# Qw11111111111/SequenceAligning

Hardware: AMD Instinct MI355X
Metric: GCUPS (affine-gap NW) at 1/2/4/8 MI355X; % of HBM roofline (higher is better)
Workload: dtype i32-exact (i16x2 packed arithmetic)

## Files before the change

### sequencealigning_amd/csrc/nw_host.cpp

```cpp
#include <hip/hip_runtime.h>

#include <algorithm>
#include <cstdlib>
#include <array>
#include <cstring>
#include <map>
#include <numeric>
#include <string>
#include <thread>
#include <unordered_set>
#include <vector>

#include "nw_host.hpp"

namespace saln {

Scoring scoring_or_default(const saln_nw_scoring *s) {
    if (!s) return Scoring{5, -4, -8, -6};
    return Scoring{s->match, s->mismatch, s->gap_open, s->gap_extend};
}

bool scores_fit_i32(const Scoring &s, uint64_t lq, uint64_t ld) {
    auto a = [](int64_t v) { return v < 0 ? -v : v; };
    const int64_t step = std::max({a(s.match), a(s.mismatch), a(s.gap_open) + a(s.gap_extend)});
// ... 225 lines not shown
        }
    return SALN_OK;
}

}

int saln::plan_create(saln_context *ctx, const uint64_t *q_off, uint64_t n_q,
                      const uint64_t *db_off, uint64_t n_db, const uint32_t *pair_q,
                      const uint32_t *pair_db, uint64_t n_pairs, int32_t mode,
                      const saln_nw_scoring *scoring, bool full_codes, saln_nw_plan **out) {
    if (!ctx || !q_off || !db_off || !out) return SALN_E_INVALID;
    *out = nullptr;
    if (mode != SALN_MODE_GLOBAL) {
        set_error("not implemented");
        return SALN_NOT_IMPLEMENTED;
    }
    const PairIndex pairs{pair_q, pair_db, n_q, n_db};
    if (!pairs.complete(n_pairs) || n_pairs > 0xFFFFFFFFull) return SALN_E_INVALID;
    HIP_TRY(hipSetDevice(ctx->device));
    const Options opts = ctx->opts.effective();
    StageClock clk(opts);
    auto *p = new saln_nw_plan;
    p->ctx = ctx;
    p->opts = opts;
    p->sc = scoring_or_default(scoring);
    p->full_codes = full_codes;
    const bool nib_on = !full_codes;
    const bool narrow = nib_on;
    for (int v = 0; v < kNumVariants; ++v) p->nib[v] = nib_on && variant_nib(v);
    p->n_pairs = n_pairs;
    p->cigar_off.resize(n_pairs + 1);
    std::vector<NwPairDesc> descs(n_pairs);
    uint64_t cig = 0;
    uint64_t memo_lq = ~0ull, memo_ld = ~0ull;
    bool memo_fit = false;
    int memo_var = 0;
    for (uint64_t k = 0; k < n_pairs; ++k) {
        uint64_t qi, di, lq, ld;
        if (!pairs.at(k, &qi, &di) ||
            !pair_lengths(q_off, db_off, qi, di, 0x7FFFFFFFull, &lq, &ld)) {
            delete p;
            return SALN_E_INVALID;
        }
        NwPairDesc &d = descs[k];
        std::memset(&d, 0, sizeof(d));
        d.q_off = q_off[qi];
        d.db_off = db_off[di];
        if (lq != memo_lq || ld != memo_ld) {
            memo_lq = lq;
            memo_ld = ld;
            memo_fit = scores_fit_i32(p->sc, lq, ld);
            memo_var = memo_fit ? choose_variant((uint32_t)lq, (uint32_t)ld, p->sc, narrow) : 0;
        }
        if (!memo_fit) {
            delete p;
            set_error("pair too long for these penalties: its scores could leave the engine's "
                      "int32 range");
            return SALN_E_INVALID;
        }
        d.len_q = (uint32_t)lq;
        d.len_db = (uint32_t)ld;
        d.pair_id = (uint32_t)k;
        d.variant = (uint32_t)memo_var;
        d.cigar_off = cig;
        p->cigar_off[k] = cig;
        cig += lq + ld;
        p->cells += lq * ld;
    }
    p->cigar_off[n_pairs] = cig;
    clk.mark("plan: descs");
    {
        const uint64_t v8_min = (uint64_t)opts[Opt::WideMinPairs];
        uint64_t wide = 0;
        for (const NwPairDesc &d : descs)
            wide += d.variant == (uint32_t)kWidePackedVariant && d.len_q > 512;
        if (wide && wide < v8_min)
            for (NwPairDesc &d : descs)
                if (d.variant == (uint32_t)kWidePackedVariant && d.len_q > 512)
                    d.variant = (uint32_t)kStripeVariant;
    }
    std::vector<uint64_t> skey(n_pairs);
    for (uint64_t k = 0; k < n_pairs; ++k) {
        const NwPairDesc &d = descs[k];
        const bool empty = d.len_q == 0 || d.len_db == 0;
        const uint64_t nch = empty ? 0 : variant_geom((int)d.variant).n_chunks(d.len_q);
        skey[k] = (uint64_t)(empty ? (uint32_t)kNumVariants : d.variant) << 56 |
                  ((~nch) & 0xFFFFFFull) << 32 | (uint32_t)~d.len_db;
    }
    std::vector<uint32_t> order;
    const bool in_order = std::is_sorted(skey.begin(), skey.end());
    if (in_order) {
        p->h_pairs = std::move(descs);
    } else {
        order.resize(n_pairs);
        std::iota(order.begin(), order.end(), 0u);
        std::sort(order.begin(), order.end(), [&](uint32_t a, uint32_t b) {
            return skey[a] != skey[b] ? skey[a] < skey[b] : a < b;
        });
        p->h_pairs.resize(n_pairs);
    }
    clk.mark("plan: sort");
    uint64_t soff = 0, ooff = 0;
    for (uint64_t r = 0; r < n_pairs; ++r) {
        NwPairDesc d = in_order ? p->h_pairs[r] : descs[order[r]];
        const bool empty = d.len_q == 0 || d.len_db == 0;
        if (!empty) {
            const Geom g = variant_geom((int)d.variant);
            d.ops_off = ooff;
            ooff += (d.len_q + d.len_db + 9) / 10 + 1;
            if (g.n_chunks(d.len_q) > 1 || d.variant == kStripeVariant) {
                soff = (soff + 3) & ~3ull;
                d.scratch_off = soff;
                soff += (uint64_t)(d.variant == kStripeVariant ? kStripeSubMax * g.n_chunks(d.len_q)
                                                                : 1) *
                        scratch_col(d.len_db);
            }
            if (p->var_count[d.variant] == 0) p->var_first[d.variant] = (uint32_t)r;
            p->var_count[d.variant]++;
            p->var_maxld[d.variant] = std::max(p->var_maxld[d.variant], d.len_db);
            p->n_fill++;
        }
        p->h_pairs[r] = d;
    }
    {
        uint64_t waves = 0, cols = 0, waves_k1 = 0;
        bool free_all = true;
        for (uint32_t r = 0; r < p->var_count[kStripeVariant]; ++r) {
            const NwPairDesc &d = p->h_pairs[p->var_first[kStripeVariant] + r];
            waves += variant_geom(kStripeVariant).n_chunks(d.len_q);
            waves_k1 += (d.len_q + 63) / 64;
            cols += d.len_q;
            free_all = free_all && sentinel_free(p->sc, d.len_q, d.len_db);
        }
        const bool wide = p->var_count[kStripeVariant] &&
                          cols / p->var_count[kStripeVariant] >= 3000;
        p->stripe_pk = waves > 0 && free_all && stripe_packed(p->sc, waves, wide, opts);
        p->stripe_rows = p->stripe_pk ? 0 : stripe_rows_k(waves_k1, opts);
        p->stripe_sub = p->stripe_rows ? 4u / (uint32_t)p->stripe_rows : 1u;
        if (p->stripe_sub != kStripeSubMax) {
            uint64_t so = 0;
            for (uint64_t r = 0; r < p->n_fill; ++r) {
                NwPairDesc &d = p->h_pairs[r];
                const Geom g = variant_geom((int)d.variant);
                if (g.n_chunks(d.len_q) > 1 || d.variant == kStripeVariant) {
                    so = (so + 3) & ~3ull;
                    d.scratch_off = so;
                    so += (uint64_t)(d.variant == kStripeVariant ? p->stripe_sub * g.n_chunks(d.len_q) : 1) *
                          scratch_col(d.len_db);
                }
            }
            soff = so;
        }
    }
    uint64_t moff = 0;
    for (int v = 0; v < kNumVariants; ++v) {
        const Geom g = variant_geom(v);
        const uint64_t lb = p->nib[v] ? g.LBn() : g.LB();
        for (uint32_t a = p->var_first[v], e = a + p->var_count[v]; a < e; a += 64) {
            const uint32_t np = std::min<uint32_t>(64, e - a);
            uint64_t rows = 0, nbm = 0, own = 0;
            for (uint32_t s = 0; s < np; ++s) {
                const NwPairDesc &d = p->h_pairs[a + s];
                rows = std::max<uint64_t>(rows, d.len_db);
                nbm = std::max<uint64_t>(nbm, g.n_blocks(d.len_q));
                own += (uint64_t)d.len_db * g.n_blocks(d.len_q) * lb;
            }
            const uint64_t packed = rows * nbm * np * lb;
            if (v == kStripeVariant) {
                const bool pk = p->stripe_pk;
                for (uint32_t s = 0; s < np; ++s) {
                    NwPairDesc &d = p->h_pairs[a + s];
                    d.mask_off = moff;
                    d.mask_rs = g.W();
                    d.mask_bs = pk ? 0u : (uint32_t)lb;
                    d.mask_cs = ((uint64_t)d.len_db + (pk ? 2 * g.G : g.G) - 1) * g.W();
                    moff += g.n_chunks(d.len_q) * d.mask_cs;
                }
            } else if (4 * packed <= 5 * own + 4096) {
                for (uint32_t s = 0; s < np; ++s) {
                    NwPairDesc &d = p->h_pairs[a + s];
                    d.mask_off = moff + s * lb;
                    d.mask_bs = (uint32_t)(np * lb);
                    d.mask_rs = nbm * np * lb;
                    d.mask_cs = (uint64_t)g.G * d.mask_bs;
                }
                moff += (packed + 255) & ~255ull;
            } else {
                for (uint32_t s = 0; s < np; ++s) {
                    NwPairDesc &d = p->h_pairs[a + s];
                    d.mask_off = moff;
                    d.mask_bs = (uint32_t)lb;
                    d.mask_rs = g.n_blocks(d.len_q) * lb;
                    d.mask_cs = (uint64_t)g.G * lb;
                    moff += ((uint64_t)d.len_db * d.mask_rs + 255) & ~255ull;
                }
            }
        }
    }
    {
        p->sync_ev.resize(3);
        for (auto &e : p->sync_ev) {
            if (hipEventCreateWithFlags(&e, hipEventDisableTiming) != hipSuccess) {
                e = nullptr;
                set_error("hipEventCreate");
                saln_nw_plan_destroy(p);
                return SALN_E_HIP;
            }
        }
    }
    clk.mark("plan: layout");
    p->plan_index.resize(n_pairs);
    for (uint64_t r = 0; r < n_pairs; ++r) p->plan_index[p->h_pairs[r].pair_id] = (uint32_t)r;
    p->mask_bytes = moff;
    p->scratch_elems = soff;
    auto fail = [&](hipError_t e, const char *what) {
        set_error(std::string(what) + ": " + hipGetErrorString(e));
        saln_nw_plan_destroy(p);
        return SALN_E_HIP;
    };
    hipError_t e;
    if (n_pairs) {
        if ((e = dev_alloc(p->ctx, (void **)&p->d_pairs, n_pairs * sizeof(NwPairDesc))) != hipSuccess)
            return fail(e, "hipMalloc(pairs)");
        clk.mark("plan: pairs alloc");
        {
            std::lock_guard<std::mutex> lk(p->ctx->staging_mu);
            void *st = nullptr;
            const size_t nb = n_pairs * sizeof(NwPairDesc);
            if ((e = pinned_staging(p->ctx, nb, &st)) != hipSuccess) return fail(e, "pinned staging");
            std::memcpy(st, p->h_pairs.data(), nb);
            if ((e = hipMemcpy(p->d_pairs, st, nb, hipMemcpyHostToDevice)) != hipSuccess)
                return fail(e, "hipMemcpy(pairs)");
        }
        if ((e = dev_alloc(p->ctx, (void **)&p->d_endh, n_pairs * sizeof(int32_t))) != hipSuccess)
            return fail(e, "hipMalloc(end)");
    }
    clk.mark("plan: pairs h2d");
    if (moff && (e = dev_alloc(p->ctx, (void **)&p->d_mask, moff + 64)) != hipSuccess)
        return fail(e, "hipMalloc(mask workspace)");
    {
        std::vector<uint2> work;
        p->work_first.assign(n_pairs + 1, 0);
        for (uint64_t r = 0; r < n_pairs; ++r) {
            NwPairDesc &d = p->h_pairs[r];
            p->work_first[r] = (uint32_t)work.size();
            if (d.variant != (uint32_t)kStripeVariant || !d.len_q || !d.len_db) continue;
            const uint32_t nch = variant_geom(kStripeVariant).n_chunks(d.len_q);
            d.reserved = (uint32_t)p->n_prog;
            p->n_prog += nch;
            for (uint32_t ch = 0; ch < nch; ++ch) work.push_back(make_uint2((uint32_t)r, ch));
        }
        p->work_first[n_pairs] = (uint32_t)work.size();
        if (!work.empty()) {
            if ((e = dev_alloc(p->ctx, (void **)&p->d_work, work.size() * sizeof(uint2))) != hipSuccess ||
                (e = hipMemcpy(p->d_work, work.data(), work.size() * sizeof(uint2),
                               hipMemcpyHostToDevice)) != hipSuccess ||
                (e = dev_alloc(p->ctx, (void **)&p->d_prog, p->n_prog * sizeof(uint32_t))) != hipSuccess ||
                (e = dev_alloc(p->ctx, (void **)&p->d_err, kErrWords * sizeof(uint32_t))) != hipSuccess ||
                (e = hipMemset(p->d_err, 0, kErrWords * sizeof(uint32_t))) != hipSuccess ||
                (e = hipMemcpy(p->d_err, std::array<uint32_t, 2>{0u, kWaitLimitDefault}.data(),
                               2 * sizeof(uint32_t), hipMemcpyHostToDevice)) != hipSuccess)
                return fail(e, "stripe work list");
            if ((e = hipMemcpy(p->d_pairs, p->h_pairs.data(), n_pairs * sizeof(NwPairDesc),
                               hipMemcpyHostToDevice)) != hipSuccess)
                return fail(e, "hipMemcpy(pairs)");
        }
    }
    clk.mark("plan: mask+work");
    if (soff && (e = dev_alloc(p->ctx, (void **)&p->d_scratch, soff * sizeof(int2))) != hipSuccess)
        return fail(e, "hipMalloc(scratch)");
    p->ops_words = ooff;
    if (ooff && (e = dev_alloc(p->ctx, (void **)&p->d_ops, ooff * sizeof(uint32_t))) != hipSuccess)
        return fail(e, "hipMalloc(op stream)");
    if ((p->var_count[kNarrowVariant] && p->nib[kNarrowVariant]) || (p->var_count[7] && p->nib[7]) ||
        (p->full_codes && (p->var_count[5] || p->var_count[7]))) {
        if ((e = dev_alloc(p->ctx, (void **)&p->d_bail[0], kBailBytes)) != hipSuccess ||
            (e = hipMemset(p->d_bail[0], 0, kBailBytes)) != hipSuccess)
            return fail(e, "table fill bail words");
    }
    {
        const int passes = (int)opts[Opt::SpecPasses];
        const uint32_t nv = p->var_count[kStripeVariant];
        std::vector<SpecPair> sp;
        std::vector<uint2> blocks;
        if (opts[Opt::Spec] != 0 && passes > 0 && nv && nv <= kSpecMaxPairs) {
            for (uint32_t r = p->var_first[kStripeVariant]; r < p->var_first[kStripeVariant] + nv; ++r) {
                const NwPairDesc &d = p->h_pairs[r];
                const uint32_t S = (d.len_q + 255) / 256;
                if (S < kSpecMinStripes || S > kSpecMaxStripes) continue;
                sp.push_back(SpecPair{r, S, (uint32_t)blocks.size(), 0});
                for (uint32_t s = 0; s < S; ++s) blocks.push_back(make_uint2((uint32_t)sp.size() - 1, s));
            }
        }
        if (!sp.empty()) {
            p->spec_pairs = (uint32_t)sp.size();
            p->spec_blocks = (uint32_t)blocks.size();
            p->spec_passes = passes;
            p->spec_strict = opts[Opt::SpecStrict] != 0;
            if ((e = dev_alloc(p->ctx, (void **)&p->d_spec_blocks, blocks.size() * sizeof(uint2))) != hipSuccess ||
                (e = hipMemcpy(p->d_spec_blocks, blocks.data(), blocks.size() * sizeof(uint2),
                               hipMemcpyHostToDevice)) != hipSuccess ||
                (e = dev_alloc(p->ctx, (void **)&p->d_spec_pairs, sp.size() * sizeof(SpecPair))) != hipSuccess ||
                (e = hipMemcpy(p->d_spec_pairs, sp.data(), sp.size() * sizeof(SpecPair),
                               hipMemcpyHostToDevice)) != hipSuccess ||
                (e = dev_alloc(p->ctx, (void **)&p->d_spec_stripes, blocks.size() * sizeof(SpecStripe))) != hipSuccess ||
                (e = dev_alloc(p->ctx, (void **)&p->d_spec_ops,
                               blocks.size() * kSpecOpsCap * sizeof(uint32_t))) != hipSuccess ||
                (e = dev_alloc(p->ctx, (void **)&p->d_spec_done, n_pairs * sizeof(uint32_t))) != hipSuccess ||
                (e = hipMemset(p->d_spec_done, 0, n_pairs * sizeof(uint32_t))) != hipSuccess)
                return fail(e, "speculative walk tables");
        }
    }
    *out = p;
    return SALN_OK;
}

extern "C" {

int saln_nw_plan_info(const saln_nw_plan *p, uint64_t *mask_bytes, uint64_t *cigar_words,
                      uint64_t *cells) {
    if (!p) return SALN_E_INVALID;
    if (mask_bytes) *mask_bytes = p->mask_bytes;
    if (cigar_words) *cigar_words = p->cigar_off.back();
    if (cells) *cells = p->cells;
    return SALN_OK;
}

int saln_nw_cigar_offsets(const saln_nw_plan *p, uint64_t *off) {
    if (!p || !off) return SALN_E_INVALID;
    std::memcpy(off, p->cigar_off.data(), p->cigar_off.size() * sizeof(uint64_t));
    return SALN_OK;
}

int saln_nw_plan_set_timing(saln_nw_plan *p, int enable) {
    if (!p) return SALN_E_INVALID;
    HIP_TRY(hipSetDevice(p->ctx->device));
    if (p->ev_used) {
        const int rc = p->resolve_events();
        if (rc != SALN_OK) return rc;
    }
    p->timing = enable != 0;
    p->ktime.clear();
    constexpr size_t kEventSets = 64;
    while (p->timing && p->ev_pool.size() < kEventSets) {
        std::array<hipEvent_t, 4> e4{};
        for (auto &e : e4) HIP_TRY(hipEventCreate(&e));
// ... 544 lines not shown
```

### sequencealigning_amd/csrc/nw_kernels.hip

```cpp
#include <hip/hip_runtime.h>

#include <algorithm>
#include <atomic>
#include <cstdlib>
#include <type_traits>
#include <utility>

#include "nw_common.hpp"
#include "nw_host.hpp"
#include "saln_options.hpp"
#include "saln.h"

namespace saln {
bool stripe_packed(const Scoring &sc, uint64_t n_waves, bool wide, const Options &o);
}

namespace saln {

template <int G>
__device__ __forceinline__ int32_t shr1(int32_t old, int32_t v) {
    static_assert(G == 16 || G == 64, "group must be a DPP row or the wave");
    if constexpr (G == 16)
        return __builtin_amdgcn_update_dpp(old, v, 0x111 , 0xf, 0xf, false);
    else
// ... 58 lines not shown
        if (st == kStM) {
            if (i == 0 && j == 0) { ev = kEvOrigin; break; }
            if (i == 0 || j == 0) { ev = kEvDead; break; }
            const bool eq = q ? q[j - 1] == d[i - 1] : (mc.byte(i, j) >> 7) != 0;
            op = eq ? SALN_CIGAR_EQ : SALN_CIGAR_X;
            const uint8_t a = mc.argmax(i - 1, j - 1);
            --i;
            --j;
            st = (a & kArgD) ? kStD : ((a & kArgI) ? kStI : kStM);
        } else if (st == kStI) {
            if (j == 0) { ev = i >= 1 ? kEvPanic : kEvDead; break; }
            if (i == 0) { ev = kEvDead; break; }
            op = SALN_CIGAR_I;
            const uint8_t b = mc.ibits(i, j);
            --j;
            st = (b & 2) ? kStM : kStI;
        } else {
            if (i == 0) { ev = j >= 1 ? kEvPanic : kEvDead; break; }
            if (j == 0) { ev = kEvDead; break; }
            op = SALN_CIGAR_D;
            const uint8_t b = mc.dbits(i, j);
            --i;
            st = (b & 2) ? kStM : kStD;
        }
        if (op == run_op && run_len) {
            ++run_len;
        } else {
            if (run_len && out) out[nops] = (run_len << 4) | run_op;
            nops += run_len ? 1 : 0;
            run_op = op;
            run_len = 1;
        }
    }
    if (run_len) {
        if (out) out[nops] = (run_len << 4) | run_op;
        ++nops;
    }
    if (ev != kEvOrigin) nops = 0;
    if (out) {
        for (uint32_t a = 0, b = nops ? nops - 1 : 0; a < b; ++a, --b) {
            const uint32_t tmp = out[a];
            out[a] = out[b];
            out[b] = tmp;
        }
    }
    return WalkOut{ev, nops};
}

__device__ WalkOut walk_first(const MaskCell &mc, uint32_t es, uint32_t ld, uint32_t lq,
                              const uint8_t *q, const uint8_t *d, uint32_t *out) {
    WalkOut w{kEvDead, 0};
    while (es) {
        const int st = first_end_state(es);
        w = walk_greedy(mc, st, ld, lq, q, d, out);
        if (w.ev != kEvDead) break;
        es = end_states_after(es, st);
    }
    return w;
}

__device__ __forceinline__ saln_nw_result make_result(int32_t hend, WalkOut w, uint32_t es) {
    saln_nw_result r;
    r.score = hend >> 1;
    r.status = (hend & 1) ? SALN_REF_PANIC_BOUNDARY : SALN_OK;
    r.cigar_len = w.nops;
    r.end_states = (uint8_t)es;
    r.printed = w.ev == kEvOrigin ? 1 : 0;
    r.flags = (w.ev == kEvPanic && !(hend & 1)) ? 2 : 0;
    r.reserved = 0;
    return r;
}

__device__ __forceinline__ void walk_pair(const NwPairDesc &p, int32_t hend,
                                       const uint8_t *__restrict__ qs,
                                       const uint8_t *__restrict__ ds,
                                       const uint8_t *__restrict__ mask, Geom geo,
                                       saln_nw_result *__restrict__ results,
                                       uint32_t *__restrict__ cigar, Scoring sc) {
    const uint32_t lq = p.len_q, ld = p.len_db;
    const MaskCell mc{mask + p.mask_off, geo, p.mask_rs, p.mask_bs, p.mask_cs, sc};
    const uint8_t es = ld == 0 ? argmax_row0(sc, lq)
                     : lq == 0 ? argmax_col0(sc, ld) : (mc.byte(ld, lq) & 7);
    const WalkOut w = walk_first(mc, es, ld, lq, qs + p.q_off, ds + p.db_off,
                                 cigar ? cigar + p.cigar_off : nullptr);
    results[p.pair_id] = make_result(hend, w, es);
}

constexpr uint32_t kOpsPerWord = 10;

template <int K, bool kNib = false, uint32_t kCols = 0>
struct WalkGeo {
    static constexpr uint32_t LB = kNib ? 4 * ((K + 3) / 4 / 2 + 1) : (K + 3) / 4 * 4;
    static constexpr uint32_t NW = 2;
    static constexpr uint32_t W = K < 16 || kNib ? 4 : 8;
    static constexpr uint32_t SB = LB == 12 ? 12 : 16;
    static constexpr uint32_t kSlotBytes = 64 * 16;
    static constexpr uint32_t kWinBytes = W * kSlotBytes;
    static constexpr uint32_t QC = kNib ? (15 + kCols + 15) / 16 : 0;
    static constexpr uint32_t kWaveLds = NW * kWinBytes + QC * kSlotBytes;
    static constexpr uint32_t kVmcnt = NW * (W - 1);
    static_assert(LB <= 16, "LDS window slots hold 16 bytes per lane");
    static_assert((NW == 2 || NW == 3) && W >= 2 && W <= 8, "8 valid bits per window");
    static_assert(!kNib || kCols > 0, "4-bit walk: the variant's query width");
};

typedef __attribute__((address_space(3))) uint8_t lds_u8;

__device__ __forceinline__ uint32_t lds_off(const lds_u8 *p) { return (uint32_t)(uintptr_t)p; }

__device__ __forceinline__ void counted_store(uint32_t *ptr, uint32_t v) {
    asm volatile("global_store_dword %0, %1, off" : : "v"(ptr), "v"(v) : "memory");
}

__host__ __device__ constexpr uint32_t next_state_raw(uint32_t st, uint32_t f) {
    const uint32_t pr = f ^ 7u;
    return st == 0 ? ((pr & 2) ? kStD : (pr & 1) ? kStI : kStM)
         : st == 1 ? ((pr & 2) ? kStM : kStI)
         : st == 2 ? ((pr & 2) ? kStM : kStD)
                   : ((pr & 4) ? kStD : (pr & 1) ? kStM : kStI);
}
__host__ __device__ constexpr uint64_t make_next_lut() {
    uint64_t l = 0;
    for (uint32_t st = 0; st < 4; ++st)
        for (uint32_t f = 0; f < 8; ++f) l |= (uint64_t)next_state_raw(st, f) << (16 * st + 2 * f);
    return l;
}
constexpr uint64_t kNextLut = make_next_lut();

typedef uint32_t u32x4 __attribute__((ext_vector_type(4)));
template <uint32_t N>
__device__ __forceinline__ u32x4 window_seg(uint32_t addr) {
    static_assert(N < 64, "vmcnt immediate");
    u32x4 v;
    asm volatile("s_waitcnt vmcnt(%2)\n\tds_read_b128 %0, %1\n\ts_waitcnt lgkmcnt(0)"
                 : "=v"(v) : "v"(addr), "n"(N) : "memory");
    return v;
}

template <typename F, uint32_t... I>
__device__ __forceinline__ void unroll_each(F &&f, std::integer_sequence<uint32_t, I...>) {
    (f(std::integral_constant<uint32_t, I>{}), ...);
}

template <int G, int K, bool kNib = false>
__device__ void walk_pack_lds(const NwPairDesc &p, int32_t hend, const uint8_t *__restrict__ mask,
                              uint32_t *__restrict__ ops_all, saln_nw_result *__restrict__ results,
                              uint32_t *__restrict__ cigar, Scoring sc, lds_u8 *win,
                              const uint8_t *__restrict__ qs) {
    using WG = WalkGeo<K, kNib, G * K>;
    constexpr Geom geo{G, K};
    constexpr uint32_t kW = WG::W, NW = WG::NW;
    constexpr uint32_t kWin = WG::kWinBytes, kSlot = WG::kSlotBytes;
    constexpr uint64_t kMask30 = (1u << 30) - 1u;
    const uint64_t rs = p.mask_rs, cs = p.mask_cs;
    const uint32_t bs = p.mask_bs;
    const uint8_t *__restrict__ m = mask + p.mask_off;
    uint32_t *out = cigar ? cigar + p.cigar_off : nullptr;
    uint32_t *const ops = ops_all + p.ops_off;
    auto boff = [&](uint32_t b) __attribute__((always_inline)) {
        if constexpr (kNib) return (uint64_t)(b * bs);
        else return (uint64_t)(b / G) * cs + (uint64_t)((b % G) * bs);
    };
    uint64_t acc = 0;
    uint32_t sh = 0, wi = 0;
    uint32_t ti = p.len_db, tj = p.len_q;
    uint32_t sidx = 3u * 16u, lsh = 0;
    uint32_t walking = 1;
    uint32_t B = (tj - 1) / K, col = (tj - 1) % K;
    uint32_t wc = B % NW;
    uint32_t valid = NW == 3 ? 0xFFFFFFu : 0xFFFFu;
    uint64_t ow0 = 0, ow1 = 0, ow2 = 0;
    auto set_ow = [&](uint32_t w, uint64_t o) __attribute__((always_inline)) {
        ow0 = w == 0 ? o : ow0;
        ow1 = w == 1 ? o : ow1;
        if constexpr (NW == 3) ow2 = w == 2 ? o : ow2;
    };
    auto get_ow = [&](uint32_t w) __attribute__((always_inline)) {
        return NW == 3 ? (w == 0 ? ow0 : w == 1 ? ow1 : ow2) : (w == 0 ? ow0 : ow1);
    };
    for (uint32_t b = 0; b < NW; ++b)
        set_ow((B + NW - b) % NW, boff(B >= b ? B - b : 0));
    const uint32_t wbase = lds_off(win) + (threadIdx.x & 63u) * 16u;
    const uint32_t qa = (uint32_t)(p.q_off & 15u);
    lds_u8 *const qlds = win + NW * kWin;
    if constexpr (kNib) {
        const uint8_t *qg = qs + (p.q_off - qa);
        const uint32_t qlast = (qa + p.len_q - 1u) / 16u;
#pragma unroll
        for (uint32_t c = 0; c < WG::QC; ++c)
            __builtin_amdgcn_global_load_lds(qg + 16u * (c < qlast ? c : qlast),
                                             (__attribute__((address_space(3))) void *)(qlds + c * kSlot),
                                             16, 0, 0);
    }
    auto qeq = [&](uint32_t j, uint32_t dch) __attribute__((always_inline)) {
        const uint32_t o = qa + j - 1u;
        return (uint32_t)qlds[(o >> 4) * kSlot + (threadIdx.x & 63u) * 16u + (o & 15u)] == dch;
    };
    constexpr uint32_t kNG = (K + 3) / 4, kCB = kNG % 2 ? 4 * (kNG / 2) + 2 : 4 * (kNG / 2);
    auto nib_bit = [](uint32_t c) __attribute__((always_inline)) {
        return ((c & 4u) << 2) | ((c & 1u) << 3) | (c & 2u) << 1;
    };
    auto end_bits = [](uint32_t n4) __attribute__((always_inline)) {
        return ((n4 >> 3) & 1u) | ((n4 & 3u) << 1);
    };
    uint32_t wl = wbase + wc * kWin;
    const uint8_t *rp = m + (uint64_t)(ti - 1) * rs;
    int32_t row = (int32_t)ti;
    const uint64_t rsW = (uint64_t)kW * rs;
    auto dma = [&](auto win_c, auto slot_c, const uint8_t *a) __attribute__((always_inline)) {
        constexpr uint32_t w = decltype(win_c)::value, s = decltype(slot_c)::value;
        __builtin_amdgcn_global_load_lds(
            a, (__attribute__((address_space(3))) void *)(win + w * kWin + s * kSlot), WG::SB, 0,
            0);
    };
    static_assert(NW == 2, "two windows: the lane's block and the one left of it");
    auto refill = [&](auto slot_c, const uint8_t *row) __attribute__((always_inline)) {
        constexpr uint32_t S = decltype(slot_c)::value;
        const bool near = walking && col < kW + 2u;
        const bool own0 = walking && wc == 0u, own1 = walking && wc == 1u;
        dma(std::integral_constant<uint32_t, 0>{}, slot_c, (own0 || near) ? row + ow0 : m);
        dma(std::integral_constant<uint32_t, 1>{}, slot_c, (own1 || near) ? row + ow1 : m);
        const uint32_t mine = 1u << (wc * 8u + S), other = 1u << ((wc ^ 1u) * 8u + S);
        valid = (valid | mine | (near ? other : 0u)) & ~(near ? 0u : other);
    };
    auto ensure = [&](auto slot_c) __attribute__((always_inline)) {
        constexpr uint32_t S = decltype(slot_c)::value;
        if (!((valid >> (wc * 8u + S)) & 1u)) {
            const uint8_t *a = rp + get_ow(wc);
            if (wc == 0) dma(std::integral_constant<uint32_t, 0>{}, slot_c, a);
            __builtin_amdgcn_sched_barrier(0);
            if (wc == 1) dma(std::integral_constant<uint32_t, 1>{}, slot_c, a);
            if constexpr (NW == 3) {
                __builtin_amdgcn_sched_barrier(0);
                if (wc == 2) dma(std::integral_constant<uint32_t, 2>{}, slot_c, a);
            }
            asm volatile("s_waitcnt vmcnt(0)" : : : "memory");
            valid |= 1u << (wc * 8u + S);
        }
    };
    auto flush = [&]() __attribute__((always_inline)) {
        counted_store(ops + wi, (uint32_t)(acc & kMask30));
        acc >>= 30;
        sh -= 30;
        ++wi;
    };
    auto cross = [&]() __attribute__((always_inline)) {
        set_ow(wc, boff(B >= NW ? B - NW : 0));
        valid &= ~(0xFFu << (wc * 8u));
        wc = wc == 0 ? NW - 1 : wc - 1;
        wl = wbase + wc * kWin;
        --B;
        col = K - 1;
    };
    auto pick = [](const u32x4 &v, uint32_t k) __attribute__((always_inline)) {
        if constexpr (WG::LB <= 8) return k == 0 ? v.x : v.y;
        else if constexpr (WG::LB <= 12) return k == 0 ? v.x : k == 1 ? v.y : v.z;
        else return k == 0 ? v.x : k == 1 ? v.y : k == 2 ? v.z : v.w;
    };
    auto iopen = [](uint32_t d) __attribute__((always_inline)) {
        return __builtin_amdgcn_ubfe((~d & 0x10101010u) * 0x00204081u, 25, 4);
    };
    auto iopen_n = [](uint32_t h) __attribute__((always_inline)) {
        return __builtin_amdgcn_ubfe((uint32_t)__umul24(~h & 0x4444u, 0x285u), 11, 4);
    };
    auto iopen_n8 = [&](uint32_t d) __attribute__((always_inline)) {
        return iopen_n(d) | (iopen_n(d >> 16) << 4);
    };
    auto iopen_mask = [&](const u32x4 &v) __attribute__((always_inline)) {
        if constexpr (kNib) {
            uint32_t pm = iopen_n8(v.x);
            if constexpr (K > 8) pm |= iopen_n8(v.y) << 8;
            if constexpr (K > 16) pm |= iopen_n8(v.z) << 16;
            return pm;
        } else {
            uint32_t pm = iopen(v.x) | (iopen(v.y) << 4);
            if constexpr (WG::LB > 8) pm |= iopen(v.z) << 8;
            if constexpr (WG::LB > 12) pm |= iopen(v.w) << 12;
            return pm;
        }
    };
    constexpr uint32_t kOnes3 = 0x09249249u;
    auto phase = [&](auto slot_c) __attribute__((always_inline)) {
        constexpr uint32_t S = decltype(slot_c)::value;
        const uint8_t *ahead = row > (int32_t)kW ? rp - rsW : m;
        if (walking) {
            ensure(slot_c);
            for (;;) {
                if (sh >= 30) flush();
                const u32x4 seg = window_seg<WG::kVmcnt>(wl + S * kSlot);
                if (sidx != 16u) {
                    uint32_t f3, eqb;
                    if constexpr (kNib) {
                        const uint32_t dw = pick(seg, col >> 3);
                        f3 = sidx == 48u ? end_bits(__builtin_amdgcn_ubfe(dw, nib_bit(col), 4))
                                         : __builtin_amdgcn_ubfe(dw, nib_bit(col) + lsh, 3);
                        const uint32_t dch = __builtin_amdgcn_ubfe(pick(seg, kCB >> 2), (kCB & 3u) * 8u, 8);
                        eqb = qeq(tj, dch) ? 1u : 0u;
                    } else {
                        const uint32_t dw = pick(seg, col >> 2), b8 = (col & 3u) * 8u;
                        f3 = __builtin_amdgcn_ubfe(dw, b8 + lsh, 3);
                        eqb = __builtin_amdgcn_ubfe(dw, b8 + 7u, 1);
                    }
                    const uint32_t nx = (uint32_t)(kNextLut >> (f3 * 2u + sidx)) & 3u;
                    acc |= (uint64_t)(nx | (eqb << 2)) << sh;
                    sh += 3;
                    sidx = nx * 16u;
                    lsh = kNib ? nx : 2u * nx + 1u;
                    const bool up = nx != kStI, left = nx != kStD;
                    ti -= up ? 1u : 0u;
                    tj -= left ? 1u : 0u;
                    const bool done = ti == 0 || tj == 0;
                    bool crossed = false;
                    if (left && !done) {
                        if (col == 0) {
                            cross();
                            crossed = true;
                        } else {
                            --col;
                        }
                    }
                    if (up || done) {
                        walking = done ? 0u : 1u;
                        break;
                    }
                    if (crossed) {
                        ensure(slot_c);
                        continue;
                    }
                }
                const uint32_t lo = col >= 8u ? col - 8u : 0u;
                const uint32_t pm = iopen_mask(seg) & ((2u << col) - 1u) & (~0u << lo);
                if (pm) {
                    const uint32_t c1 = 31u - (uint32_t)__builtin_clz(pm), n = col - c1;
                    uint32_t eqb;
                    if constexpr (kNib)
                        eqb = qeq(tj - n, __builtin_amdgcn_ubfe(pick(seg, kCB >> 2), (kCB & 3u) * 8u, 8))
                                  ? 1u : 0u;
                    else
                        eqb = __builtin_amdgcn_ubfe(pick(seg, c1 >> 2), (c1 & 3u) * 8u + 7u, 1);
                    acc |= (uint64_t)((kOnes3 & ((1u << (3u * n)) - 1u)) | (eqb << (3u * n + 2u)))
                           << sh;
                    sh += 3u * (n + 1u);
                    sidx = 0;
                    lsh = kNib ? 0u : 1u;
                    ti -= 1;
                    tj -= n + 1u;
                    const bool done = ti == 0 || tj == 0;
                    if (!done) {
                        if (c1 == 0) cross();
                        else col = c1 - 1u;
                    }
                    walking = done ? 0u : 1u;
                    break;
                }
                const uint32_t n = col - lo + 1u;
                acc |= (uint64_t)(kOnes3 & ((1u << (3u * n)) - 1u)) << sh;
                sh += 3u * n;
                tj -= n;
                if (tj == 0) {
                    walking = 0;
                    break;
                }
                if (lo == 0) cross();
                else col = lo - 1u;
                ensure(slot_c);
            }
        }
        if (sh >= 30) flush();
        refill(slot_c, ahead);
        rp -= rs;
        --row;
    };
    unroll_each([&](auto slot_c) __attribute__((always_inline)) {
        constexpr uint32_t S = decltype(slot_c)::value;
        refill(slot_c, ti > S ? rp - (uint64_t)S * rs : m);
    }, std::make_integer_sequence<uint32_t, kW>{});
    while (walking) unroll_each(phase, std::make_integer_sequence<uint32_t, kW>{});
    const uint32_t st = sidx / 16u;
    int ev, bst;
    if (st == kStM && ti == 0 && tj == 0) {
        ev = kEvOrigin;
    } else {
        if (st == kStM) {
            const uint8_t a = ti == 0 ? argmax_row0_walk(sc, tj) : argmax_col0_walk(sc, ti);
            bst = (a & kArgD) ? kStD : ((a & kArgI) ? kStI : kStM);
        } else if (st == kStI) {
            bst = (ibits_col1_walk(sc, ti) & 2) ? kStM : kStI;
        } else {
            bst = (dbits_row1_walk(sc, tj) & 2) ? kStM : kStD;
        }
        if (bst == kStD && ti == 0 && tj >= 1) ev = kEvPanic;
        else if (bst == kStI && tj == 0 && ti >= 1) ev = kEvPanic;
        else ev = kEvDead;
    }
    uint32_t es;
    if constexpr (kNib) {
        const uint32_t c = (p.len_q - 1) % K, b = (p.len_q - 1) / K;
        const uint32_t w = *reinterpret_cast<const uint32_t *>(
            m + (uint64_t)(p.len_db - 1) * rs + boff(b) + 4u * (c >> 3));
        es = ~end_bits(__builtin_amdgcn_ubfe(w, nib_bit(c), 4)) & 7u;
    } else {
        es = (m[geo.cell(p.len_db, p.len_q, rs, bs, cs)] ^ 0x7Fu) & 7u;
    }
    uint32_t nops = 0;
    bool retried = false;
    if (!kNib && ev == kEvDead) {
        const uint32_t rest = end_states_after(es, first_end_state(es));
        if (rest) {
            const MaskCell mc{m, geo, rs, bs, cs, sc};
            const WalkOut w = walk_first(mc, rest, p.len_db, p.len_q, nullptr, nullptr, out);
            ev = w.ev;
            nops = w.nops;
            retried = true;
        }
    }
    if (ev == kEvOrigin && !retried) {
        const uint32_t nrec = wi * kOpsPerWord + sh / 3;
        if (sh) counted_store(ops + wi, (uint32_t)(acc & kMask30));
        if (sh > 30) counted_store(ops + wi + 1, (uint32_t)(acc >> 30));
        asm volatile("s_waitcnt vmcnt(0)" : : : "memory");
        constexpr uint32_t kSlots = 0x09249249u;
        constexpr uint32_t kOpOf = (SALN_CIGAR_X << 12) | (SALN_CIGAR_D << 8) |
                                   (SALN_CIGAR_I << 4) | SALN_CIGAR_EQ;
        static_assert(SALN_CIGAR_X < 16 && SALN_CIGAR_EQ < 16, "4-bit CIGAR ops");
        uint32_t run_cls = 4u, run_len = 0;
        int32_t w = (int32_t)((nrec - 1u) / kOpsPerWord);
        uint32_t word = ops[w], nxt = w > 0 ? ops[w - 1] : 0u;
        uint32_t top = (nrec - 1u) % kOpsPerWord;
        for (; w >= 0; --w, top = kOpsPerWord - 1) {
            const uint32_t cur = word;
            word = nxt;
            nxt = w >= 2 ? ops[w - 2] : 0u;
            const uint32_t s0 = cur & kSlots, s1 = (cur >> 1) & kSlots, e = (cur >> 2) & kSlots;
            const uint32_t xm = ~(s0 | s1 | e) & kSlots;
            const uint32_t c0 = s0 | xm, c1 = s1 | xm;
            const uint32_t chg = ((c0 ^ (c0 >> 3)) | (c1 ^ (c1 >> 3))) & kSlots &
                                 ((1u << (3u * top)) - 1u);
            int32_t pos = (int32_t)top;
            for (;;) {
                const uint32_t below = chg & ((1u << (3u * (uint32_t)pos)) - 1u);
                const int32_t b = below ? (31 - __builtin_clz(below)) / 3 : -1;
                const uint32_t cls = ((c0 >> (3u * (uint32_t)pos)) & 1u) |
                                     (((c1 >> (3u * (uint32_t)pos)) & 1u) << 1);
                const uint32_t len = (uint32_t)(pos - b);
                if (cls != run_cls) {
                    if (run_len) {
                        if (out) out[nops] = (run_len << 4) | ((kOpOf >> (4u * run_cls)) & 15u);
                        ++nops;
                    }
                    run_cls = cls;
                    run_len = 0;
                }
                run_len += len;
                if (b < 0) break;
                pos = b;
            }
        }
        if (run_len) {
            if (out) out[nops] = (run_len << 4) | ((kOpOf >> (4u * run_cls)) & 15u);
            ++nops;
        }
    }
    results[p.pair_id] = make_result(hend, WalkOut{ev, nops}, es);
}

template <int G, int K, bool kNib = false>
constexpr uint32_t tb_lds_threads() { return kNib ? 128u : 256u; }
template <int G, int K, bool kNib>
__global__ __launch_bounds__(256) void nw_traceback_lds_kernel(
    const NwPairDesc *__restrict__ pairs, uint32_t first, uint32_t n,
    const uint8_t *__restrict__ mask, const int32_t *__restrict__ end_h,
    uint32_t *__restrict__ ops, saln_nw_result *__restrict__ results,
    uint32_t *__restrict__ cigar, Scoring sc, const uint8_t *__restrict__ qs) {
    constexpr uint32_t kWave = WalkGeo<K, kNib, G * K>::kWaveLds;
    __shared__ __attribute__((aligned(16))) uint8_t win_all[tb_lds_threads<G, K, kNib>() / 64u * kWave];
    __builtin_amdgcn_s_setprio(3);
    lds_u8 *win = (lds_u8 *)(win_all + (threadIdx.x / 64u) * kWave);
    const uint32_t stride = gridDim.x * blockDim.x;
    bool later = false;
    for (uint32_t rel = blockIdx.x * blockDim.x + threadIdx.x; rel < n; rel += stride) {
        if (later) __builtin_amdgcn_s_setprio(1);
        later = true;
        const uint32_t idx = first + rel;
        const NwPairDesc p = pairs[idx];
        walk_pack_lds<G, K, kNib>(p, end_h[idx], mask, ops, results, cigar, sc, win, qs);
    }
}

__global__ __launch_bounds__(256) void nw_traceback_kernel(
    const NwPairDesc *__restrict__ pairs, uint32_t first, uint32_t n,
    const uint8_t *__restrict__ qs, const uint8_t *__restrict__ ds,
    const uint8_t *__restrict__ mask, const int32_t *__restrict__ end_h,
    saln_nw_result *__restrict__ results, uint32_t *__restrict__ cigar, Scoring sc,
    GeomTable gt) {
    const uint32_t idx = first + blockIdx.x * blockDim.x + threadIdx.x;
    if (idx >= first + n) return;
    const NwPairDesc p = pairs[idx];
    const Geom geo = gt.g[p.variant];
    walk_pair(p, p.len_q && p.len_db ? end_h[idx] : hs_boundary_end(sc, p.len_q, p.len_db), qs,
              ds, mask, geo, results, cigar, sc);
}

__global__ __launch_bounds__(256) void nw_next_event_kernel(
    const NwPairDesc *__restrict__ pairs, uint32_t n, const uint8_t *__restrict__ mask,
    const saln_nw_result *__restrict__ results, Scoring sc, GeomTable gt,
    uint8_t *__restrict__ next) {
    const uint32_t idx = blockIdx.x * blockDim.x + threadIdx.x;
    if (idx >= n) return;
    const NwPairDesc p = pairs[idx];
    const saln_nw_result r = results[p.pair_id];
    uint8_t out = kNextNone;
    if (r.printed && p.len_q && p.len_db) {
        if (!sentinel_free(sc, p.len_q, p.len_db)) {
            out = kNextHost;
        } else {
            const MaskCell mc{mask + p.mask_off, gt.g[p.variant], p.mask_rs, p.mask_bs, p.mask_cs, sc};
            int st = first_end_state(r.end_states);
            const uint32_t rest = end_states_after(r.end_states, st);
            int ast = rest ? first_end_state(rest) : -1;
            uint32_t ai = p.len_db, aj = p.len_q;
            uint32_t i = p.len_db, j = p.len_q;
            for (uint32_t guard = 0; !(i == 0 && j == 0) && guard <= p.len_q + p.len_db; ++guard) {
                int ps[3];
                uint32_t pi[3], pj[3];
                int np = 0;
                auto push = [&](int s2, uint32_t i2, uint32_t j2) {
                    ps[np] = s2;
                    pi[np] = i2;
                    pj[np] = j2;
                    ++np;
                };
                if (i == 0 || j == 0) break;
                if (st == kStM) {
                    const uint8_t a = mc.argmax(i - 1, j - 1);
                    if (a & kArgM) push(kStM, i - 1, j - 1);
                    if (a & kArgI) push(kStI, i - 1, j - 1);
                    if (a & kArgD) push(kStD, i - 1, j - 1);
                } else if (st == kStI) {
                    const uint8_t b = mc.ibits(i, j);
                    if (b & 1) push(kStI, i, j - 1);
                    if (b & 2) push(kStM, i, j - 1);
                } else {
                    const uint8_t b = mc.dbits(i, j);
                    if (b & 1) push(kStD, i - 1, j);
                    if (b & 2) push(kStM, i - 1, j);
                }
                if (np == 0) break;
                if (np >= 2) {
                    ast = ps[np - 2];
                    ai = pi[np - 2];
                    aj = pj[np - 2];
                }
                st = ps[np - 1];
                i = pi[np - 1];
                j = pj[np - 1];
            }
            if (!(i == 0 && j == 0 && st == kStM)) {
                out = kNextHost;
            } else if (ast >= 0) {
                const WalkOut w = walk_greedy(mc, ast, ai, aj, nullptr, nullptr, nullptr);
                out = w.ev == kEvOrigin ? kNextBlock : w.ev == kEvPanic ? kNextPanic : kNextHost;
            }
        }
    }
    next[p.pair_id] = out;
}

hipError_t launch_next_event(const NwPairDesc *pairs, uint32_t n, const uint8_t *mask,
                             const saln_nw_result *results, Scoring sc, uint8_t *next,
                             hipStream_t stream) {
    if (!n) return hipSuccess;
    GeomTable gt;
    for (int v = 0; v < kNumVariants; ++v) gt.g[v] = variant_geom(v);
    nw_next_event_kernel<<<dim3((n + 255) / 256), dim3(256), 0, stream>>>(pairs, n, mask, results,
                                                                       sc, gt, next);
    return hipGetLastError();
}

constexpr int32_t kCoopLine = 256;
constexpr int32_t kCoopSlack = 64;

template <int NWV, int kLay, bool kSpec = false>
__global__ __launch_bounds__(64 * NWV) void nw_traceback_coop_kernel(
    const NwPairDesc *__restrict__ pairs, uint32_t first, const uint8_t *__restrict__ mask,
    const int32_t *__restrict__ end_h, saln_nw_result *__restrict__ results,
    uint32_t *__restrict__ cigar, Scoring sc, int32_t kCoopRows,
    const uint8_t *__restrict__ qs, const uint8_t *__restrict__ ds, SpecArgs sa) {
    static_assert(kLay == 1 || kLay == 2, "round 1's skewed i32 stripe layout is retired");
    constexpr bool kPk = kLay == 1;
    constexpr int32_t kSkew = kLay == 1 ? 127 : 0;
    extern __shared__ __attribute__((aligned(16))) uint8_t win[];
    int32_t *req = reinterpret_cast<int32_t *>(win + (kCoopRows + kSkew + 1) * kCoopLine);
    uint8_t *qwin = win + (kCoopRows + kSkew + 1) * kCoopLine + 16;
    uint8_t *dwin = qwin + 272;
    const int32_t lane = (int32_t)threadIdx.x % 64, wv = (int32_t)threadIdx.x / 64;
    uint32_t idx = first + blockIdx.x;
    SpecStripe *rec = nullptr;
    int32_t ei = 0, ej = 0, ek = 0, s_id = 0;
    if constexpr (kSpec) {
        const uint2 b = sa.blocks[blockIdx.x];
        const SpecPair sp = sa.pairs[b.x];
        idx = sp.plan_idx;
        s_id = (int32_t)b.y;
        rec = sa.stripes + sp.stripe_base + b.y;
    } else if (sa.done && sa.done[idx]) {
        return;
    }
    const NwPairDesc p = pairs[idx];
    const uint8_t *__restrict__ m = mask + p.mask_off;
    if constexpr (kSpec) {
        const int32_t lqp = (int32_t)p.len_q, ldp = (int32_t)p.len_db;
        const int32_t par = (sa.pass - 1) & 1, cur = sa.pass & 1;
        if (sa.entry_s1 && s_id == sa.entry_s1 - 1) {
            ei = rec[1].out_i[par];
            ej = rec[1].out_j[par];
            ek = rec[1].out_k[par];
        } else if (s_id == (lqp - 1) / kCoopLine) {
            ei = ldp;
            ej = lqp;
            ek = kSpecEnd;
        } else if (sa.pass == 1) {
            ej = kCoopLine * (s_id + 1);
            ei = (int32_t)min((int64_t)ldp, max((int64_t)1, (int64_t)ej * ldp / lqp));
            ek = kSpecM;
        } else {
            ei = rec[1].out_i[par];
            ej = rec[1].out_j[par];
            ek = rec[1].out_k[par];
        }
        if (ek >= kSpecEv) {
// ... 2582 lines not shown
```

Before: 2728.

## Use 32-bit mask offsets and bit-parallel nibble scan in LDS traceback walk

Switches the traceback walker's mask addressing from 64-bit pointers to 32-bit offsets off a single base pointer, and adds host checks so no pair or packed group spans more than 4 GB of mask. It also replaces the per-nibble insertion-open scan with a dword-wide swizzle plus alignbit over a larger run window, defers block crossing to the loop head, and makes the LDS window base wave-uniform via readfirstlane. The aim is fewer VGPRs and 64-bit address ops in the serial walk loop. In exchange, very large pairs are now rejected, and the reworked column and crossing logic carries correctness risk.

```diff
diff --git a/sequencealigning_amd/csrc/nw_host.cpp b/sequencealigning_amd/csrc/nw_host.cpp
--- a/sequencealigning_amd/csrc/nw_host.cpp
+++ b/sequencealigning_amd/csrc/nw_host.cpp
@@ -401,6 +401,7 @@
             soff = so;
         }
     }
+    constexpr uint64_t kWalkSpanMax = 0xFFFFFFFFull;
     uint64_t moff = 0;
     for (int v = 0; v < kNumVariants; ++v) {
         const Geom g = variant_geom(v);
@@ -425,7 +426,7 @@
                     d.mask_cs = ((uint64_t)d.len_db + (pk ? 2 * g.G : g.G) - 1) * g.W();
                     moff += g.n_chunks(d.len_q) * d.mask_cs;
                 }
-            } else if (4 * packed <= 5 * own + 4096) {
+            } else if (4 * packed <= 5 * own + 4096 && packed <= kWalkSpanMax) {
                 for (uint32_t s = 0; s < np; ++s) {
                     NwPairDesc &d = p->h_pairs[a + s];
                     d.mask_off = moff + s * lb;
@@ -441,6 +442,11 @@
                     d.mask_bs = (uint32_t)lb;
                     d.mask_rs = g.n_blocks(d.len_q) * lb;
                     d.mask_cs = (uint64_t)g.G * lb;
+                    if ((uint64_t)d.len_db * d.mask_rs > kWalkSpanMax) {
+                        set_error("pair too large: its traceback mask would pass 4 GB");
+                        saln_nw_plan_destroy(p);
+                        return SALN_E_INVALID;
+                    }
                     moff += ((uint64_t)d.len_db * d.mask_rs + 255) & ~255ull;
                 }
             }
diff --git a/sequencealigning_amd/csrc/nw_kernels.hip b/sequencealigning_amd/csrc/nw_kernels.hip
--- a/sequencealigning_amd/csrc/nw_kernels.hip
+++ b/sequencealigning_amd/csrc/nw_kernels.hip
@@ -234,14 +234,14 @@
     constexpr uint32_t kW = WG::W, NW = WG::NW;
     constexpr uint32_t kWin = WG::kWinBytes, kSlot = WG::kSlotBytes;
     constexpr uint64_t kMask30 = (1u << 30) - 1u;
-    const uint64_t rs = p.mask_rs, cs = p.mask_cs;
+    const uint32_t rs = (uint32_t)p.mask_rs, cs = (uint32_t)p.mask_cs;
     const uint32_t bs = p.mask_bs;
     const uint8_t *__restrict__ m = mask + p.mask_off;
     uint32_t *out = cigar ? cigar + p.cigar_off : nullptr;
     uint32_t *const ops = ops_all + p.ops_off;
     auto boff = [&](uint32_t b) __attribute__((always_inline)) {
-        if constexpr (kNib) return (uint64_t)(b * bs);
-        else return (uint64_t)(b / G) * cs + (uint64_t)((b % G) * bs);
+        if constexpr (kNib) return b * bs;
+        else return (b / G) * cs + (b % G) * bs;
     };
     uint64_t acc = 0;
     uint32_t sh = 0, wi = 0;
@@ -251,8 +251,8 @@
     uint32_t B = (tj - 1) / K, col = (tj - 1) % K;
     uint32_t wc = B % NW;
     uint32_t valid = NW == 3 ? 0xFFFFFFu : 0xFFFFu;
-    uint64_t ow0 = 0, ow1 = 0, ow2 = 0;
-    auto set_ow = [&](uint32_t w, uint64_t o) __attribute__((always_inline)) {
+    uint32_t ow0 = 0, ow1 = 0, ow2 = 0;
+    auto set_ow = [&](uint32_t w, uint32_t o) __attribute__((always_inline)) {
         ow0 = w == 0 ? o : ow0;
         ow1 = w == 1 ? o : ow1;
         if constexpr (NW == 3) ow2 = w == 2 ? o : ow2;
@@ -286,29 +286,29 @@
         return ((n4 >> 3) & 1u) | ((n4 & 3u) << 1);
     };
     uint32_t wl = wbase + wc * kWin;
-    const uint8_t *rp = m + (uint64_t)(ti - 1) * rs;
+    uint32_t rp = (ti - 1) * rs;
     int32_t row = (int32_t)ti;
-    const uint64_t rsW = (uint64_t)kW * rs;
-    auto dma = [&](auto win_c, auto slot_c, const uint8_t *a) __attribute__((always_inline)) {
+    const uint32_t rsW = kW * rs;
+    auto dma = [&](auto win_c, auto slot_c, uint32_t off) __attribute__((always_inline)) {
         constexpr uint32_t w = decltype(win_c)::value, s = decltype(slot_c)::value;
         __builtin_amdgcn_global_load_lds(
-            a, (__attribute__((address_space(3))) void *)(win + w * kWin + s * kSlot), WG::SB, 0,
-            0);
+            m + off, (__attribute__((address_space(3))) void *)(win + w * kWin + s * kSlot),
+            WG::SB, 0, 0);
     };
     static_assert(NW == 2, "two windows: the lane's block and the one left of it");
-    auto refill = [&](auto slot_c, const uint8_t *row) __attribute__((always_inline)) {
+    auto refill = [&](auto slot_c, uint32_t row) __attribute__((always_inline)) {
         constexpr uint32_t S = decltype(slot_c)::value;
-        const bool near = walking && col < kW + 2u;
+        const bool near = walking && (int32_t)col < (int32_t)(kW + 2u);
         const bool own0 = walking && wc == 0u, own1 = walking && wc == 1u;
-        dma(std::integral_constant<uint32_t, 0>{}, slot_c, (own0 || near) ? row + ow0 : m);
-        dma(std::integral_constant<uint32_t, 1>{}, slot_c, (own1 || near) ? row + ow1 : m);
+        dma(std::integral_constant<uint32_t, 0>{}, slot_c, (own0 || near) ? row + ow0 : 0u);
+        dma(std::integral_constant<uint32_t, 1>{}, slot_c, (own1 || near) ? row + ow1 : 0u);
         const uint32_t mine = 1u << (wc * 8u + S), other = 1u << ((wc ^ 1u) * 8u + S);
         valid = (valid | mine | (near ? other : 0u)) & ~(near ? 0u : other);
     };
     auto ensure = [&](auto slot_c) __attribute__((always_inline)) {
         constexpr uint32_t S = decltype(slot_c)::value;
         if (!((valid >> (wc * 8u + S)) & 1u)) {
-            const uint8_t *a = rp + get_ow(wc);
+            const uint32_t a = rp + get_ow(wc);
             if (wc == 0) dma(std::integral_constant<uint32_t, 0>{}, slot_c, a);
             __builtin_amdgcn_sched_barrier(0);
             if (wc == 1) dma(std::integral_constant<uint32_t, 1>{}, slot_c, a);
@@ -342,38 +342,48 @@
     auto iopen = [](uint32_t d) __attribute__((always_inline)) {
         return __builtin_amdgcn_ubfe((~d & 0x10101010u) * 0x00204081u, 25, 4);
     };
-    auto iopen_n = [](uint32_t h) __attribute__((always_inline)) {
-        return __builtin_amdgcn_ubfe((uint32_t)__umul24(~h & 0x4444u, 0x285u), 11, 4);
-    };
-    auto iopen_n8 = [&](uint32_t d) __attribute__((always_inline)) {
-        return iopen_n(d) | (iopen_n(d >> 16) << 4);
-    };
     auto iopen_mask = [&](const u32x4 &v) __attribute__((always_inline)) {
-        if constexpr (kNib) {
-            uint32_t pm = iopen_n8(v.x);
-            if constexpr (K > 8) pm |= iopen_n8(v.y) << 8;
-            if constexpr (K > 16) pm |= iopen_n8(v.z) << 16;
-            return pm;
+        uint32_t pm = iopen(v.x) | (iopen(v.y) << 4);
+        if constexpr (WG::LB > 8) pm |= iopen(v.z) << 8;
+        if constexpr (WG::LB > 12) pm |= iopen(v.w) << 12;
+        return pm;
+    };
+    auto iopen_sw = [](uint32_t d) __attribute__((always_inline)) {
+        const uint32_t x = ~d & 0x44444444u, t = (x ^ (x >> 4)) & 0x00400040u;
+        return x ^ (t | (t << 4));
+    };
+    auto iopen_win = [&](const u32x4 &v) __attribute__((always_inline)) {
+        static_assert(!kNib || (4u * K) / 32u < WG::LB / 4u, "column K-1's dword");
+        const uint32_t e = 4u * col + 4u, d = e >> 5;
+        uint32_t hi, lo;
+        if constexpr (WG::LB <= 8) {
+            hi = d == 0 ? v.x : v.y;
+            lo = d == 0 ? ~0u : v.x;
         } else {
-            uint32_t pm = iopen(v.x) | (iopen(v.y) << 4);
-            if constexpr (WG::LB > 8) pm |= iopen(v.z) << 8;
-            if constexpr (WG::LB > 12) pm |= iopen(v.w) << 12;
-            return pm;
-        }
-    };
+            hi = d == 0 ? v.x : d == 1 ? v.y : v.z;
+            lo = d == 0 ? ~0u : d == 1 ? v.x : v.y;
+        }
+        return __builtin_amdgcn_alignbit(iopen_sw(hi), iopen_sw(lo), e);
+    };
+    auto pick_col = [](const u32x4 &v, uint32_t c) __attribute__((always_inline)) {
+        if constexpr (WG::LB <= 8) return c < 8u ? v.x : v.y;
+        else return c < 8u ? v.x : c < 16u ? v.y : v.z;
+    };
+    constexpr uint32_t kRun = kNib ? 8u : 9u;
     constexpr uint32_t kOnes3 = 0x09249249u;
     auto phase = [&](auto slot_c) __attribute__((always_inline)) {
         constexpr uint32_t S = decltype(slot_c)::value;
-        const uint8_t *ahead = row > (int32_t)kW ? rp - rsW : m;
+        const uint32_t ahead = row > (int32_t)kW ? rp - rsW : 0u;
         if (walking) {
-            ensure(slot_c);
             for (;;) {
+                if ((int32_t)col < 0) cross();
+                ensure(slot_c);
                 if (sh >= 30) flush();
                 const u32x4 seg = window_seg<WG::kVmcnt>(wl + S * kSlot);
                 if (sidx != 16u) {
                     uint32_t f3, eqb;
                     if constexpr (kNib) {
-                        const uint32_t dw = pick(seg, col >> 3);
+                        const uint32_t dw = pick_col(seg, col);
                         f3 = sidx == 48u ? end_bits(__builtin_amdgcn_ubfe(dw, nib_bit(col), 4))
                                          : __builtin_amdgcn_ubfe(dw, nib_bit(col) + lsh, 3);
                         const uint32_t dch = __builtin_amdgcn_ubfe(pick(seg, kCB >> 2), (kCB & 3u) * 8u, 8);
@@ -392,28 +402,26 @@
                     ti -= up ? 1u : 0u;
                     tj -= left ? 1u : 0u;
                     const bool done = ti == 0 || tj == 0;
-                    bool crossed = false;
-                    if (left && !done) {
-                        if (col == 0) {
-                            cross();
-                            crossed = true;
-                        } else {
-                            --col;
-                        }
-                    }
+                    col -= left ? 1u : 0u;
                     if (up || done) {
                         walking = done ? 0u : 1u;
                         break;
                     }
-                    if (crossed) {
-                        ensure(slot_c);
-                        continue;
+                    if ((int32_t)col < 0) continue;
+                }
+                const uint32_t lo = col >= kRun - 1u ? col - (kRun - 1u) : 0u;
+                uint32_t pm;
+                if constexpr (kNib) pm = iopen_win(seg);
+                else pm = iopen_mask(seg) & ((2u << col) - 1u) & (~0u << lo);
+                if (pm) {
+                    uint32_t c1, n;
+                    if constexpr (kNib) {
+                        n = (uint32_t)__builtin_clz(pm) >> 2;
+                        c1 = col - n;
+                    } else {
+                        c1 = 31u - (uint32_t)__builtin_clz(pm);
+                        n = col - c1;
                     }
-                }
-                const uint32_t lo = col >= 8u ? col - 8u : 0u;
-                const uint32_t pm = iopen_mask(seg) & ((2u << col) - 1u) & (~0u << lo);
-                if (pm) {
-                    const uint32_t c1 = 31u - (uint32_t)__builtin_clz(pm), n = col - c1;
                     uint32_t eqb;
                     if constexpr (kNib)
                         eqb = qeq(tj - n, __builtin_amdgcn_ubfe(pick(seg, kCB >> 2), (kCB & 3u) * 8u, 8))
@@ -427,12 +435,8 @@
                     lsh = kNib ? 0u : 1u;
                     ti -= 1;
                     tj -= n + 1u;
-                    const bool done = ti == 0 || tj == 0;
-                    if (!done) {
-                        if (c1 == 0) cross();
-                        else col = c1 - 1u;
-                    }
-                    walking = done ? 0u : 1u;
+                    col = c1 - 1u;
+                    walking = ti == 0 || tj == 0 ? 0u : 1u;
                     break;
                 }
                 const uint32_t n = col - lo + 1u;
@@ -443,19 +447,16 @@
                     walking = 0;
                     break;
                 }
-                if (lo == 0) cross();
-                else col = lo - 1u;
-                ensure(slot_c);
-            }
-        }
-        if (sh >= 30) flush();
+                col = lo - 1u;
+            }
+        }
         refill(slot_c, ahead);
         rp -= rs;
         --row;
     };
     unroll_each([&](auto slot_c) __attribute__((always_inline)) {
         constexpr uint32_t S = decltype(slot_c)::value;
-        refill(slot_c, ti > S ? rp - (uint64_t)S * rs : m);
+        refill(slot_c, ti > S ? rp - S * rs : 0u);
     }, std::make_integer_sequence<uint32_t, kW>{});
     while (walking) unroll_each(phase, std::make_integer_sequence<uint32_t, kW>{});
     const uint32_t st = sidx / 16u;
@@ -482,14 +483,14 @@
             m + (uint64_t)(p.len_db - 1) * rs + boff(b) + 4u * (c >> 3));
         es = ~end_bits(__builtin_amdgcn_ubfe(w, nib_bit(c), 4)) & 7u;
     } else {
-        es = (m[geo.cell(p.len_db, p.len_q, rs, bs, cs)] ^ 0x7Fu) & 7u;
+        es = (m[geo.cell(p.len_db, p.len_q, p.mask_rs, bs, p.mask_cs)] ^ 0x7Fu) & 7u;
     }
     uint32_t nops = 0;
     bool retried = false;
     if (!kNib && ev == kEvDead) {
         const uint32_t rest = end_states_after(es, first_end_state(es));
         if (rest) {
-            const MaskCell mc{m, geo, rs, bs, cs, sc};
+            const MaskCell mc{m, geo, p.mask_rs, bs, p.mask_cs, sc};
             const WalkOut w = walk_first(mc, rest, p.len_db, p.len_q, nullptr, nullptr, out);
             ev = w.ev;
             nops = w.nops;
@@ -557,7 +558,7 @@
     constexpr uint32_t kWave = WalkGeo<K, kNib, G * K>::kWaveLds;
     __shared__ __attribute__((aligned(16))) uint8_t win_all[tb_lds_threads<G, K, kNib>() / 64u * kWave];
     __builtin_amdgcn_s_setprio(3);
-    lds_u8 *win = (lds_u8 *)(win_all + (threadIdx.x / 64u) * kWave);
+    lds_u8 *win = (lds_u8 *)(win_all + __builtin_amdgcn_readfirstlane(threadIdx.x / 64u) * kWave);
     const uint32_t stride = gridDim.x * blockDim.x;
     bool later = false;
     for (uint32_t rel = blockIdx.x * blockDim.x + threadIdx.x; rel < n; rel += stride) {
```

After: 2724. About the same (-0.1%).
